# lighttransport/nanort

Measured on NVIDIA H100. Metric: Mrays/sec (primary+1-bounce AO), higher is better.
Workload: dtype f32

## Files before the change

### nanort_b200/csrc/bake.cu

```cuda
#include <algorithm>
#include <mutex>
#include <string>

#include "../../include/nanort_b200_bake.h"
#include "common.cuh"
#include "scan.cuh"
#include "wavefront.cuh"

namespace nrt {

int launch_traverse_texels(const Accel *a, const TexelRays &rays, size_t n, const TexelStore &store, Hit16 *d_by_ray,
                           uint32_t flags, cudaStream_t s);
int launch_traverse_bake(const Accel *a, const BakeAoRays &rays, size_t n, float *d_accum, unsigned long long *d_occluded,
                         uint32_t flags, cudaStream_t s);

namespace {

__global__ void __launch_bounds__(256)
    scatter_texels_kernel(const Hit16 *__restrict__ by_ray, uint32_t n, TexelRays rays, TexelStore store) {
  const uint32_t i = blockIdx.x * blockDim.x + threadIdx.x;
  const bool active = i < n;
  Hit16 h = {0.0f, 0.0f, 1.0e30f, 0xFFFFFFFFu};
  uint32_t texel = 0;
  if (active) {
// ... 3 lines not shown
  store(active, texel, h.t, h.u, h.v, h.prim_id, 1.0e30f);
}

__global__ void __launch_bounds__(256)
    covered_flags_kernel(const Hit16 *__restrict__ rec, uint32_t n, uint32_t n_prims, uint32_t *__restrict__ flags,
                         unsigned long long *info) {
  const uint32_t i = blockIdx.x * blockDim.x + threadIdx.x;
  if (i >= n) return;
  const uint32_t p = rec[i].prim_id;
  flags[i] = p != 0xFFFFFFFFu ? 1u : 0u;
  if (p != 0xFFFFFFFFu && p >= n_prims) info[1] = 1ull;
}

__global__ void __launch_bounds__(256)
    compact_texels_kernel(const Hit16 *__restrict__ rec, uint32_t n, const uint32_t *__restrict__ offs,
                          uint32_t *__restrict__ list, unsigned long long *info) {
  const uint32_t i = blockIdx.x * blockDim.x + threadIdx.x;
  if (i >= n) return;
  const bool covered = rec[i].prim_id != 0xFFFFFFFFu;
  if (covered) list[offs[i]] = i;
  if (i == n - 1) info[0] = (unsigned long long)offs[i] + (covered ? 1ull : 0ull);
}

__global__ void __launch_bounds__(256) bake_rays_kernel(BakeAoRays rays, uint32_t n, Ray36 *__restrict__ out) {
  const uint32_t i = blockIdx.x * blockDim.x + threadIdx.x;
  if (i >= n) return;
  Ray36 r;
  uint32_t texel;
  rays.load(i, r.org[0], r.org[1], r.org[2], r.dir[0], r.dir[1], r.dir[2], r.min_t, r.max_t, &texel);
  r.type = 0;
  out[i] = r;
}

uint32_t scan_launches(uint32_t n) {
  const uint32_t tiles = (n + kScanTile - 1) / kScanTile;
  return n == 0 ? 0u : tiles > 1 ? 2u + scan_launches(tiles) : 1u;
}

}

bool is_triangle_accel(const Accel *a) {
  return a->prim_kind == 0 && !a->d_prim_boxes && a->d_faces && a->d_verts && a->d_pair && a->d_tris_cm;
}

int bake_prepare(Accel *a, const void *d_records, uint32_t n, const char *who, cudaStream_t s, uint32_t **list,
                 uint32_t *n_cov, uint32_t *launches) {
  uint32_t *offs = static_cast<uint32_t *>(a->d_wave);
  *list = offs + n;
  uint32_t *scratch = *list + n;
  unsigned long long *info = reinterpret_cast<unsigned long long *>(a->d_counters) + 2;
  const Hit16 *rec = static_cast<const Hit16 *>(d_records);
  NRT_CUDA(cudaMemsetAsync(info, 0, 2 * sizeof(unsigned long long), s));
  covered_flags_kernel<<<(n + 255) / 256, 256, 0, s>>>(rec, n, a->n_prims, offs, info);
  NRT_CUDA(cudaGetLastError());
  if (const int rc = exclusive_scan_u32_async(offs, offs, n, scratch, s)) return rc;
  compact_texels_kernel<<<(n + 255) / 256, 256, 0, s>>>(rec, n, offs, *list, info);
  NRT_CUDA(cudaGetLastError());
  *launches += 2 + scan_launches(n);
  unsigned long long h[2] = {0, 0};
  NRT_CUDA(cudaMemcpyAsync(h, info, sizeof(h), cudaMemcpyDeviceToHost, s));
  NRT_CUDA(cudaStreamSynchronize(s));
  if (h[1]) {
    set_error(std::string(who) + ": a record's prim_id is not a face of the world accel");
    return NRT_ERR_INVALID;
  }
  *n_cov = (uint32_t)h[0];
  return NRT_OK;
}

}
// ... 240 lines not shown
```

### nanort_b200/csrc/bdpt.cu

```cuda
#include <algorithm>
#include <mutex>
#include <string>

#include "../../include/nanort_b200_scene_bdpt.h"
#include "common.cuh"
#include "radix_sort.cuh"
#include "scan.cuh"
#include "scene.cuh"
#include "wavefront.cuh"

namespace nrt {

int launch_traverse_bdpt_bounce(const Accel *a, const bd::BounceRays &rays, const bd::BounceEpilogue &epi,
                                const unsigned long long *d_count, size_t capacity, uint32_t flags, cudaStream_t s);
int launch_traverse_bdpt_connect(const Accel *a, const bd::ConnRays &rays, const bd::ConnEpilogue &epi,
                                 const unsigned long long *d_count, size_t capacity, uint32_t flags, cudaStream_t s);

namespace {

using namespace bd;

constexpr size_t kWaveBudget = (size_t)512 << 20;

__device__ __forceinline__ void emissive_flag(const Scene &sc, uint32_t id, uint32_t *flag, unsigned long long *info) {
// ... 527 lines not shown
  const uint32_t slot = conns[i].slot, el = conns[i].el, l = el >> 16;
  const size_t ie = (size_t)slot * sp.stride + (el & 0xFFFFu) - 1, il = (size_t)slot * sp.stride + l - 1;
  const float3 pe = f3(sp.eye[ie].position), pl = f3(sp.light[il].position);
  float3 to;
  float dist;
  conn_ray(pe, pl, to, dist);
  const float3 ge = g.geo_normal(sv.eye_inst[ie], sp.eye[ie].prim_id);
  const float3 gl = l == 1 ? g.geo_normal(sv.light_pair[2 * (size_t)slot], sv.light_pair[2 * (size_t)slot + 1])
                           : g.geo_normal(sv.light_inst[il], sp.light[il].prim_id);
  const float3 o = LiftedOrigin{ge}(pe, to);
  Ray36 r;
  r.org[0] = o.x, r.org[1] = o.y, r.org[2] = o.z;
  r.dir[0] = to.x, r.dir[1] = to.y, r.dir[2] = to.z;
  r.min_t = kEps;
  r.max_t = SceneSpawn::plane_max_t(pe.x, pe.y, pe.z, o.x, o.y, o.z, to.x, to.y, to.z, dist, gl.x, gl.y, gl.z);
  r.type = 0;
  rays[i] = r;
}

__global__ void __launch_bounds__(256)
    scene_conn_g_kernel(Conn *__restrict__ conns, uint32_t n, Subpaths sp, const Ray36 *__restrict__ rays,
                        const SceneHit32 *__restrict__ hits, const uint8_t *__restrict__ mask) {
  const uint32_t i = blockIdx.x * blockDim.x + threadIdx.x;
  if (i >= n) return;
  Conn &c = conns[i];
  const uint32_t slot = c.slot, el = c.el;
  const nrt_bdpt_vertex &ev = sp.eye[(size_t)slot * sp.stride + (el & 0xFFFFu) - 1];
  const nrt_bdpt_vertex &lv = sp.light[(size_t)slot * sp.stride + (el >> 16) - 1];
  float3 to;
  float dist;
  conn_ray(f3(ev.position), f3(lv.position), to, dist);
  const bool blocked = mask[i] && hits[i].t < rays[i].max_t;
  conn_finish(c, blocked ? 0.0f : g_term(to, dist, f3(ev.norm), f3(lv.norm)));
}

uint32_t scan_launches(uint32_t n) {
  const uint32_t tiles = (n + kScanTile - 1) / kScanTile;
  return n == 0 ? 0u : tiles > 1 ? 2u + scan_launches(tiles) : 1u;
}

uint32_t max_conns(uint32_t B) { return B * (B + 1) / 2; }

struct Out {
  nrt_bdpt_vertex *eye, *light;
  uint32_t *n_eye, *n_light;
  float *rgb;
  uint32_t *eye_inst, *light_inst, *light_pair;
};

int check_common(const nrt_bdpt_params &p, const char *who) {
  auto bad = [&](const char *why) {
    set_error(std::string(who) + ": " + why);
    return NRT_ERR_INVALID;
  };
  if (p.flags & ~(uint32_t)NRT_TRAVERSE_CONFORMANCE)
    return bad("flags other than NRT_TRAVERSE_CONFORMANCE (calcG needs the nearest distance: no ANY_HIT)");
  if (p.width == 0 || p.height == 0 || p.spp == 0 || p.n_shards == 0 || p.shard >= p.n_shards || p.tile_w == 0 ||
      p.tile_h == 0 || (p.tile_w % 8) != 0 || (p.tile_h % 4) != 0)
    return bad("bad image, sample or tile parameters");
  if ((uint64_t)p.sample0 + p.spp > p.spp_total) return bad("sample0 + spp > spp_total");
  if (p.max_bounces == 0 || p.max_bounces > 64) return bad("max_bounces must lie in [1, 64]");
  return NRT_OK;
}

int check_params(const Accel *a, const nrt_bdpt_params *pp, const char *who) {
  auto bad = [&](const char *why) {
    set_error(std::string(who) + ": " + why);
    return NRT_ERR_INVALID;
  };
  if (!a || !pp) return bad("NULL argument");
  const nrt_bdpt_params &p = *pp;
// ... 521 lines not shown
```

### nanort_b200/csrc/render.cu

```cuda
#include <algorithm>
#include <mutex>
#include <string>

#include "common.cuh"
#include "wavefront.cuh"

namespace nrt {

namespace {

__global__ void __launch_bounds__(256)
    gen_primary_kernel(nrt_ao_params p, unsigned long long slot0, uint32_t count, Wave w,
                       unsigned long long *counters ) {
  uint32_t i = blockIdx.x * blockDim.x + threadIdx.x;
  bool valid = false;
  if (i < count) {
    uint32_t pix, smp;
    if (!slot_to_pixel(p, slot0 + i, pix, smp)) {
      w.pix[i] = 0xFFFFFFFFu;
      w.org_tmin[i] = make_float4(0.f, 0.f, 0.f, 0.f);
      w.dir_tmax[i] = make_float4(0.f, 0.f, -1.f, -1.f);
    } else {
      valid = true;
      smp += p.sample0;
      float dx, dy, dz;
      camera_ray(p.cam, p.width, p.height, p.seed, pix, smp, dx, dy, dz);
      w.pix[i] = pix;
      w.org_tmin[i] = make_float4(p.cam[0], p.cam[1], p.cam[2], p.ray_min_t);
      w.dir_tmax[i] = make_float4(dx, dy, dz, p.ray_max_t);
    }
  }
  const unsigned m = __ballot_sync(0xFFFFFFFFu, valid);
  if ((threadIdx.x & 31) == 0 && m) atomicAdd(counters + 1, (unsigned long long)__popc(m));
}

__global__ void __launch_bounds__(256)
    gen_ao_kernel(nrt_ao_params p, unsigned long long slot0, uint32_t count, Wave w,
// ... 27 lines not shown
    w.ao_dir_tmax[j] = d4;
    w.ao_pix[j] = pix;
  }
}

__global__ void __launch_bounds__(256)
    face_normals_kernel(const float *__restrict__ verts, const uint32_t *__restrict__ faces, uint32_t n,
                        float4 *__restrict__ out) {
  const uint32_t i = blockIdx.x * blockDim.x + threadIdx.x;
  if (i >= n) return;
  float nx, ny, nz, a2;
  geometric_normal(verts, faces, i, nx, ny, nz, a2);
  out[i] = make_float4(nx, ny, nz, 0.0f);
}

__global__ void __launch_bounds__(256)
    accumulate_ao_kernel(Wave w, const unsigned long long *__restrict__ counters, float *__restrict__ accum,
                         unsigned long long *totals ) {
  const unsigned long long n = counters[0];
  const unsigned long long i = (unsigned long long)blockIdx.x * blockDim.x + threadIdx.x;
  bool occluded = false;
  if (i < n) {
    occluded = w.ao_hits[i].prim_id != 0xFFFFFFFFu;
    if (!occluded) atomicAdd(accum + w.ao_pix[i], 1.0f);
  }
  const unsigned m = __ballot_sync(0xFFFFFFFFu, occluded);
  if ((threadIdx.x & 31) == 0 && m) atomicAdd(totals + 1, (unsigned long long)__popc(m));
  if (i == 0) {
    atomicAdd(totals + 0, n);
    atomicAdd(totals + 2, counters[1]);
  }
}

__global__ void fold_wave_counters_kernel(const unsigned long long *counters, unsigned long long *totals) {
  totals[0] += counters[0];
  totals[2] += counters[1];
}

__global__ void __launch_bounds__(256)
    soa_to_aos_kernel(const float4 *__restrict__ org_tmin, const float4 *__restrict__ dir_tmax,
                      const unsigned long long *n_ptr, unsigned long long n, Ray36 *__restrict__ out, uint32_t type) {
  if (n_ptr) n = *n_ptr;
  const unsigned long long i = (unsigned long long)blockIdx.x * blockDim.x + threadIdx.x;
  if (i >= n) return;
  const float4 o = org_tmin[i], d = dir_tmax[i];
  Ray36 r;
  r.org[0] = o.x;
  r.org[1] = o.y;
  r.org[2] = o.z;
  r.dir[0] = d.x;
  r.dir[1] = d.y;
  r.dir[2] = d.z;
  r.min_t = o.w;
  r.max_t = d.w;
  r.type = type;
  out[i] = r;
}

}

int launch_traverse_soa_devcount(const Accel *a, const float4 *d_org_tmin, const float4 *d_dir_tmax,
                                 const unsigned long long *d_count, size_t capacity, Hit16 *d_hits,
                                 const TraceOptions16 &opt, uint32_t flags, cudaStream_t s);
int launch_traverse_camera_fused(Accel *a, const Wave &w, const nrt_ao_params &p, unsigned long long slot0, size_t count,
                                 const float4 *d_face_n, float *d_accum, unsigned long long *d_wave_counters,
                                 const TraceOptions16 &opt, uint32_t flags, cudaStream_t s);
int launch_traverse_ao_fused(const Accel *a, const Wave &w, const unsigned long long *d_count, size_t capacity,
                             float *d_accum, unsigned long long *d_totals, const TraceOptions16 &opt, uint32_t flags,
                             cudaStream_t s);

}

using namespace nrt;

static unsigned long long valid_slots(const nrt_ao_params &p, unsigned long long s0, uint32_t count) {
  const unsigned long long per_tile = (unsigned long long)p.tile_w * p.tile_h * p.spp;
  const uint32_t tiles_x = (p.width + p.tile_w - 1) / p.tile_w;
  unsigned long long total = 0;
  for (unsigned long long k = s0 / per_tile; k < (s0 + count) / per_tile; k++) {
    const unsigned long long tile = k * p.n_shards + p.shard;
    const uint32_t tx = (uint32_t)(tile % tiles_x), ty = (uint32_t)(tile / tiles_x);
    const uint32_t x0 = tx * p.tile_w, y0 = ty * p.tile_h;
    if (x0 >= p.width || y0 >= p.height) continue;
    const uint32_t wv = p.width - x0 < p.tile_w ? p.width - x0 : p.tile_w;
    const uint32_t hv = p.height - y0 < p.tile_h ? p.height - y0 : p.tile_h;
    total += (unsigned long long)wv * hv * p.spp;
  }
  return total;
}

static int run_ao_pass(const nrt_accel *h, const nrt_ao_params *pp, float *d_accum, nrt_ao_result *res, void *stream,
                       Ray36 *dump_primary, Ray36 *dump_ao, uint64_t *n_ao_out) {
  if (!h || !pp || !d_accum) {
    set_error("nrt_render_ao_device: NULL argument");
    return NRT_ERR_INVALID;
  }
  Accel *a = const_cast<Accel *>(reinterpret_cast<const Accel *>(h));
  nrt_ao_params p = *pp;
  if (p.width == 0 || p.height == 0 || p.spp == 0 || p.n_shards == 0 || p.shard >= p.n_shards || p.tile_w == 0 ||
      p.tile_h == 0 || (p.tile_w % 8) != 0 || (p.tile_h % 4) != 0) {
    set_error("nrt_render_ao_device: bad parameters (tiles must be multiples of 8x4 pixels)");
    return NRT_ERR_INVALID;
  }
  if (!a->d_pair || !a->d_tris_cm || !a->d_faces) {
    set_error("nrt_render_ao_device: the AO pass needs a triangle accel");
    return NRT_ERR_INVALID;
  }
  NRT_DEVICE(a->device);
  std::lock_guard<std::mutex> lock(a->host_mu);
  cudaStream_t s = static_cast<cudaStream_t>(stream);
  if (const int rc = wait_previous_pass(a, s)) return rc;
  const RecordOnExit pass_done{a->pass_done, s};
  if (const int rc = ensure_face_normals(a, s)) return rc;
  const uint32_t tiles_x = (p.width + p.tile_w - 1) / p.tile_w, tiles_y = (p.height + p.tile_h - 1) / p.tile_h;
  const uint32_t n_tiles = tiles_x * tiles_y;
  const uint32_t my_tiles = n_tiles > p.shard ? (n_tiles - p.shard + p.n_shards - 1) / p.n_shards : 0;
  const unsigned long long per_tile = (unsigned long long)p.tile_w * p.tile_h * p.spp;
  const unsigned long long total_slots = (unsigned long long)my_tiles * per_tile;

  const unsigned long long kMaxWave = 16ull << 20;
  unsigned long long tiles_per_wave = kMaxWave / per_tile;
  if (tiles_per_wave == 0) tiles_per_wave = 1;
  const unsigned long long cap = std::min<unsigned long long>(total_slots, tiles_per_wave * per_tile);
  const size_t per_ray = 2 * sizeof(float4) + sizeof(Hit16) + 4 + 2 * sizeof(float4) + 4 + sizeof(Hit16);
  const size_t need = (size_t)cap * per_ray + 256;
  if (const int rc = grow_wave(a, need)) return rc;
  Wave w;
  {
    char *b = static_cast<char *>(a->d_wave);
    w.org_tmin = reinterpret_cast<float4 *>(b);
    b += cap * sizeof(float4);
    w.dir_tmax = reinterpret_cast<float4 *>(b);
    b += cap * sizeof(float4);
    w.ao_org_tmin = reinterpret_cast<float4 *>(b);
    b += cap * sizeof(float4);
    w.ao_dir_tmax = reinterpret_cast<float4 *>(b);
    b += cap * sizeof(float4);
    w.hits = reinterpret_cast<Hit16 *>(b);
    b += cap * sizeof(Hit16);
    w.ao_hits = reinterpret_cast<Hit16 *>(b);
    b += cap * sizeof(Hit16);
    w.pix = reinterpret_cast<uint32_t *>(b);
    b += cap * 4;
    w.ao_pix = reinterpret_cast<uint32_t *>(b);
  }
  unsigned long long *wave_ctr = reinterpret_cast<unsigned long long *>(a->d_counters) + 2;
  unsigned long long *totals = reinterpret_cast<unsigned long long *>(a->d_counters) + 4;
  NRT_CUDA(cudaMemsetAsync(totals, 0, 3 * sizeof(unsigned long long), s));

  TraceOptions16 opt = default_trace_options();
  std::vector<cudaEvent_t> ev;
  cudaEvent_t e_begin = nullptr, e_end = nullptr;
  if (res) {
    NRT_CUDA(cudaEventCreate(&e_begin));
    NRT_CUDA(cudaEventCreate(&e_end));
    NRT_CUDA(cudaEventRecord(e_begin, s));
  }
  uint32_t launches = 0, trav_launches = 0;
  unsigned long long dumped_ao = 0, valid_primaries_host = 0;
  const bool fused = !dump_primary && !dump_ao && !(p.flags & NRT_AO_UNFUSED);
  if (!fused && (p.flags & NRT_AO_PACKED_TILES)) {
    set_error("nrt_render_ao_device: NRT_AO_PACKED_TILES needs the fused pass");
    return NRT_ERR_INVALID;
  }
  const uint32_t trav_flags = p.flags & 0xFFFFu;
  int rc = NRT_OK;
  for (unsigned long long s0 = 0; s0 < total_slots && rc == NRT_OK; s0 += cap) {
    const uint32_t count = (uint32_t)std::min<unsigned long long>(cap, total_slots - s0);
    const uint32_t grid = (count + 255) / 256;
    if (cudaMemsetAsync(wave_ctr, 0, 2 * sizeof(unsigned long long), s) != cudaSuccess) {
      rc = NRT_ERR_CUDA;
      break;
    }
    if (!fused) {
      gen_primary_kernel<<<grid, 256, 0, s>>>(p, s0, count, w, wave_ctr);
      launches++;
    }
    cudaEvent_t t0 = nullptr, t1 = nullptr, t2 = nullptr, t3 = nullptr;
    if (res) {
      cudaError_t ee = cudaEventCreate(&t0);
      if (ee == cudaSuccess) ee = cudaEventCreate(&t1);
      if (ee == cudaSuccess) ee = cudaEventCreate(&t2);
      if (ee == cudaSuccess) ee = cudaEventCreate(&t3);
      ev.push_back(t0);
      ev.push_back(t1);
      ev.push_back(t2);
      ev.push_back(t3);
      if (ee != cudaSuccess) {
        rc = cuda_fail(ee, "cudaEventCreate", __FILE__, __LINE__);
        break;
      }
    }
    if (fused) {
      if (res) cudaEventRecord(t0, s);
      rc = launch_traverse_camera_fused(a, w, p, s0, count, a->d_face_n, d_accum, wave_ctr, opt, trav_flags, s);
      if (rc != NRT_OK) break;
      if (res) {
        cudaEventRecord(t1, s);
        cudaEventRecord(t2, s);
      }
      rc = launch_traverse_ao_fused(a, w, wave_ctr, count, d_accum, totals, opt, trav_flags, s);
      if (rc != NRT_OK) break;
      if (res) cudaEventRecord(t3, s);
      fold_wave_counters_kernel<<<1, 1, 0, s>>>(wave_ctr, totals);
      launches += 3;
      trav_launches += 2;
      valid_primaries_host += valid_slots(p, s0, count);
    } else {
      if (dump_primary) {
        soa_to_aos_kernel<<<grid, 256, 0, s>>>(w.org_tmin, w.dir_tmax, nullptr, count, dump_primary + s0, 1u);
        launches++;
      }
      if (res) cudaEventRecord(t0, s);
      rc = launch_traverse_soa(a, w.org_tmin, w.dir_tmax, count, w.hits, opt, trav_flags, s);
      if (rc != NRT_OK) break;
      if (res) cudaEventRecord(t1, s);
      launches++;
      trav_launches++;
      gen_ao_kernel<<<grid, 256, 0, s>>>(p, s0, count, w, a->d_face_n, d_accum, wave_ctr);
      launches++;
      if (dump_ao) {
        unsigned long long n_wave = 0;
        soa_to_aos_kernel<<<grid, 256, 0, s>>>(w.ao_org_tmin, w.ao_dir_tmax, wave_ctr, 0, dump_ao + dumped_ao, 2u);
        launches++;
        cudaMemcpyAsync(&n_wave, wave_ctr, sizeof(n_wave), cudaMemcpyDeviceToHost, s);
        cudaStreamSynchronize(s);
        dumped_ao += n_wave;
      }
      if (res) cudaEventRecord(t2, s);
      rc = launch_traverse_soa_devcount(a, w.ao_org_tmin, w.ao_dir_tmax, wave_ctr, count, w.ao_hits, opt, trav_flags, s);
      if (rc != NRT_OK) break;
      if (res) cudaEventRecord(t3, s);
      launches++;
      trav_launches++;
      accumulate_ao_kernel<<<grid, 256, 0, s>>>(w, wave_ctr, d_accum, totals);
      launches++;
    }
    if (cudaGetLastError() != cudaSuccess) rc = NRT_ERR_CUDA;
// ... 73 lines not shown
```

### nanort_b200/csrc/scan.cuh

```cuda
#pragma once
#include "common.cuh"

namespace nrt {

constexpr int kScanBlock = 256;
constexpr int kScanItems = 8;
constexpr int kScanTile = kScanBlock * kScanItems;

static __global__ void scan_tiles_kernel(const uint32_t *__restrict__ in, uint32_t *__restrict__ out, uint32_t n,
                                         uint32_t *__restrict__ tile_sums) {
  __shared__ uint32_t warp_sums[kScanBlock / 32];
  const uint32_t base = blockIdx.x * kScanTile + threadIdx.x * kScanItems;
  uint32_t v[kScanItems];
  uint32_t sum = 0;
#pragma unroll
  for (int k = 0; k < kScanItems; k++) {
    uint32_t i = base + k;
    v[k] = i < n ? in[i] : 0u;
    sum += v[k];
  }
  uint32_t inc = sum;
  const int lane = threadIdx.x & 31, wid = threadIdx.x >> 5;
#pragma unroll
  for (int o = 1; o < 32; o <<= 1) {
// ... 44 lines not shown
  NRT_CUDA(cudaMalloc(&d_sums, sizeof(uint32_t) * (size_t)(tiles + 1)));
  scan_tiles_kernel<<<tiles, kScanBlock, 0, s>>>(d_in, d_out, n, d_sums);
  NRT_CUDA(cudaGetLastError());
  int rc = NRT_OK;
  if (tiles > 1) {
    uint32_t t2 = 0;
    rc = exclusive_scan_u32(d_sums, d_sums, tiles, total ? &t2 : nullptr, s);
    if (rc == NRT_OK) {
      add_tile_offsets_kernel<<<tiles, kScanBlock, 0, s>>>(d_out, n, d_sums);
      if (cudaGetLastError() != cudaSuccess) rc = NRT_ERR_CUDA;
    }
    if (total) *total = t2;
  } else if (total) {
    if (cudaMemcpyAsync(total, d_sums, sizeof(uint32_t), cudaMemcpyDeviceToHost, s) != cudaSuccess ||
        cudaStreamSynchronize(s) != cudaSuccess)
      rc = NRT_ERR_CUDA;
  }
  if (cudaStreamSynchronize(s) != cudaSuccess) rc = NRT_ERR_CUDA;
  cudaFree(d_sums);
  return rc;
}

static inline size_t scan_scratch_words(uint32_t n) {
  size_t total = 0;
  while (n > 1) {
    uint32_t tiles = (n + kScanTile - 1) / kScanTile;
    total += tiles + 1;
    if (tiles <= 1) break;
    n = tiles;
  }
  return total + 4;
}

static int exclusive_scan_u32_async(const uint32_t *d_in, uint32_t *d_out, uint32_t n, uint32_t *d_scratch,
                                    cudaStream_t s) {
  if (n == 0) return NRT_OK;
  uint32_t tiles = (n + kScanTile - 1) / kScanTile;
  scan_tiles_kernel<<<tiles, kScanBlock, 0, s>>>(d_in, d_out, n, d_scratch);
  NRT_CUDA(cudaGetLastError());
  if (tiles > 1) {
    int rc = exclusive_scan_u32_async(d_scratch, d_scratch, tiles, d_scratch + tiles + 1, s);
    if (rc != NRT_OK) return rc;
    add_tile_offsets_kernel<<<tiles, kScanBlock, 0, s>>>(d_out, n, d_scratch);
    NRT_CUDA(cudaGetLastError());
  }
  return NRT_OK;
}

}
```

### nanort_b200/csrc/traverse.cu

```cuda
#include <float.h>
#include <math_constants.h>

#include "common.cuh"
#include "trav_common.cuh"
#include "wavefront.cuh"
#include "traverse3.cuh"

namespace nrt {

struct AosRays {
  static constexpr int kPayloadWords = 0;
  static constexpr bool kSharedOrigin = false;
  const Ray36 *rays;
  __device__ __forceinline__ void load(size_t i, float &ox, float &oy, float &oz, float &dx, float &dy,
                                       float &dz, float &tmin, float &tmax, uint32_t * = nullptr) const {
    const float *p = reinterpret_cast<const float *>(rays + i);
    ox = __ldcs(p + 0);
    oy = __ldcs(p + 1);
    oz = __ldcs(p + 2);
    dx = __ldcs(p + 3);
    dy = __ldcs(p + 4);
    dz = __ldcs(p + 5);
    tmin = __ldcs(p + 6);
    tmax = __ldcs(p + 7);
// ... 58 lines not shown
    best.v = 0.0f;
    best.prim = 0xFFFFFFFFu;
    reference_walk(nodes, c, min_t, max_t, PackedTriLeaf{tris, c, opt, best}, COUNT ? visits : nullptr);
    if (hits) write_result(hits, mask, i, best, max_t);
  }
  if (COUNT) {
    for (int o = 16; o > 0; o >>= 1) {
      visits[0] += __shfl_down_sync(FULL_MASK, visits[0], o);
      visits[1] += __shfl_down_sync(FULL_MASK, visits[1], o);
    }
    if ((threadIdx.x & 31) == 0) {
      atomicAdd(counts + 0, visits[0]);
      atomicAdd(counts + 1, visits[1]);
    }
  }
}

static int g_sm_count[64] = {0};
int device_sm_count(int device) {
  if (device < 0 || device >= 64) return 132;
  if (g_sm_count[device] == 0) {
    int v = 0;
    if (cudaDeviceGetAttribute(&v, cudaDevAttrMultiProcessorCount, device) != cudaSuccess || v <= 0) v = 132;
    g_sm_count[device] = v;
  }
  return g_sm_count[device];
}

typedef Policy3<10, 24, true, 8, false, 2> DefaultPolicy;
typedef Policy3<9, 32, true, 12, true, 3> CameraPolicy;
typedef PacketPolicy<7, 2> CameraPacketPolicy;
typedef Policy3<10, 20, false, 12, false, 3> IncoherentPolicy;
typedef Policy3<9, 32, false, 12, true, 3> IncoherentCameraPolicy;
typedef Policy3<8, 24, false, 8, true, 2> PathRadiancePolicy;
constexpr size_t kPair128MaxBytes = (size_t)38 << 20;
constexpr size_t kCameraRelMaxBytes = (size_t)24 << 20;

template <class Rays, int DEPTH, bool COUNT, class P, class Epi>
static cudaError_t launch_fast3(const Accel *a, Rays rays, size_t n, Epi epi, const TraceOptions16 &opt,
                                uint32_t flags, unsigned long long *cursor, unsigned long long *d_counts,
                                const unsigned long long *n_ptr, cudaStream_t s) {
  const int sms = device_sm_count(a->device);
  const size_t warps_per_block = kTraverseBlock / 32;
  size_t grid = (size_t)sms * P::kMinBlocks;
  const size_t need_blocks = ((n + 31) / 32 + warps_per_block - 1) / warps_per_block;
  if (grid > need_blocks) grid = need_blocks;
  if (grid == 0) grid = 1;
  const void *nodes = Rays::kSharedOrigin ? static_cast<const void *>(a->d_pair_rel)
                     : P::kPair128        ? static_cast<const void *>(a->d_pair)
                                          : static_cast<const void *>(a->d_wide);
  const TriCM *tris = Rays::kSharedOrigin ? a->d_tris_rel : a->d_tris_cm;
  traverse_fast3_kernel<Rays, DEPTH, COUNT, P, Epi><<<(unsigned)grid, kTraverseBlock, 0, s>>>(
      nodes, tris, rays, n, epi, opt, flags, cursor, d_counts, n_ptr);
  return cudaGetLastError();
}

static bool needs_deep_stack(const Accel *a) { return a->stats.max_tree_depth + 2 > 64u; }

template <class Rays, bool COUNT, class P, class Epi>
static int launch_fast3_cursor(const Accel *a, Rays rays, size_t n, Epi epi, const TraceOptions16 &opt, uint32_t flags,
                               unsigned long long *d_counts, const unsigned long long *n_ptr, cudaStream_t s,
                               unsigned long long *cursor) {
  NRT_CUDA(cudaMemsetAsync(cursor, 0, sizeof(unsigned long long), s));
  cudaError_t e;
  if (needs_deep_stack(a))
    e = launch_fast3<Rays, 512, COUNT, P>(a, rays, n, epi, opt, flags, cursor, d_counts, n_ptr, s);
// ... 105 lines not shown
template <int DEPTH>
static cudaError_t launch_packet(const Accel *a, CameraRays rays, size_t n, const PrimaryToAoEpilogue &epi,
                                 const TraceOptions16 &opt, uint32_t flags, unsigned long long *cursor, cudaStream_t s) {
  typedef CameraUnits<CameraPacketPolicy::kRays> Units;
  const Units units(epi.p);
  const size_t n_units = units.count(n);
  const size_t warps_per_block = kTraverseBlock / 32;
  size_t grid = (size_t)device_sm_count(a->device) * CameraPacketPolicy::kMinBlocks;
  const size_t need_blocks = (n_units + warps_per_block - 1) / warps_per_block;
  if (grid > need_blocks) grid = need_blocks;
  traverse_packet_kernel<CameraRays, Units, DEPTH, CameraPacketPolicy, PrimaryToAoEpilogue>
      <<<(unsigned)grid, kTraverseBlock, 0, s>>>(a->d_pair_rel, a->d_tris_rel, rays, units, n_units, n, epi, opt, flags,
                                                 cursor);
  return cudaGetLastError();
}

static int launch_packet_any(const Accel *a, CameraRays rays, size_t n, const PrimaryToAoEpilogue &epi,
                             const TraceOptions16 &opt, uint32_t flags, cudaStream_t s) {
  if (!a->d_pair_rel || !a->d_tris_rel) {
    set_error("traverse: this accel has no camera-relative traversal layout");
    return NRT_ERR_INVALID;
  }
  return a->ring.run(s, [&](uint32_t k) {
    unsigned long long *cursor = reinterpret_cast<unsigned long long *>(a->d_counters) + 16 + k;
    NRT_CUDA(cudaMemsetAsync(cursor, 0, sizeof(unsigned long long), s));
    const cudaError_t e = needs_deep_stack(a) ? launch_packet<512>(a, rays, n, epi, opt, flags, cursor, s)
                                              : launch_packet<64>(a, rays, n, epi, opt, flags, cursor, s);
    NRT_CUDA(e);
    return NRT_OK;
  });
}

int launch_traverse_camera_fused(Accel *a, const Wave &w, const nrt_ao_params &p, unsigned long long slot0, size_t count,
                                 const float4 *d_face_n, float *d_accum, unsigned long long *d_wave_counters,
                                 const TraceOptions16 &opt, uint32_t flags, cudaStream_t s) {
  PrimaryToAoEpilogue epi{p, w, d_face_n, d_accum, d_wave_counters};
  if (count == 0) return NRT_OK;
  if (a->n_wide * sizeof(PairNode) > kPair128MaxBytes)
    return launch_fast3_any<CameraRaysAbs, false, IncoherentCameraPolicy>(a, CameraRaysAbs(p, slot0), count, epi, opt, flags,
                                                                          nullptr, nullptr, s);
  if (2 * (a->n_wide * sizeof(PairNode) + (size_t)a->n_prims * sizeof(TriCM)) > kCameraRelMaxBytes)
    return launch_fast3_any<CameraRaysAbs, false, CameraPolicy>(a, CameraRaysAbs(p, slot0), count, epi, opt, flags, nullptr,
                                                                nullptr, s);
  const int rc = camera_relative_layout(a, p.cam, s);
  if (rc != NRT_OK) return rc;
  return launch_packet_any(a, CameraRays(p, slot0), count, epi, opt, flags, s);
}

int launch_traverse_ao_fused(const Accel *a, const Wave &w, const unsigned long long *d_count, size_t capacity,
                             float *d_accum, unsigned long long *d_totals, const TraceOptions16 &opt, uint32_t flags,
                             cudaStream_t s) {
  AoAccumulateEpilogue epi{w.ao_pix, d_accum, d_totals};
  if (flags & NRT_TRAVERSE_ANY_HIT)
    return launch_fused<AnyHit<AoAccumulateEpilogue>, IncoherentPolicy>(a, SoaRays{w.ao_org_tmin, w.ao_dir_tmax}, capacity, d_count,
                                                                        AnyHit<AoAccumulateEpilogue>(epi), opt, flags, s);
  return launch_fused<AoAccumulateEpilogue, IncoherentPolicy>(a, SoaRays{w.ao_org_tmin, w.ao_dir_tmax}, capacity, d_count, epi,
                                                              opt, flags, s);
}

int launch_traverse_path_radiance(const Accel *a, const PathShadeEpilogue &epi, const unsigned long long *d_count,
                                  size_t capacity, const TraceOptions16 &opt, uint32_t flags, cudaStream_t s) {
  return launch_fused<PathShadeEpilogue, PathRadiancePolicy>(
      a, SoaRays{epi.q.org_tmin[epi.in], epi.q.dir_tmax[epi.in]}, capacity, d_count, epi, opt, flags, s);
}

int launch_traverse_lightmap_radiance(const Accel *a, const LightmapShadeEpilogue &epi, const unsigned long long *d_count,
                                      size_t capacity, const TraceOptions16 &opt, uint32_t flags, cudaStream_t s) {
  return launch_fused<LightmapShadeEpilogue, PathRadiancePolicy>(
      a, SoaRays{epi.q.org_tmin[epi.in], epi.q.dir_tmax[epi.in]}, capacity, d_count, epi, opt, flags, s);
}

int launch_traverse_path_shadow(const Accel *a, const PathQueues &q, const unsigned long long *d_count,
                                size_t capacity, float *d_accum, const TraceOptions16 &opt, uint32_t flags,
                                cudaStream_t s) {
  ShadowAccumulateEpilogue epi{q.sh_contrib_pix, d_accum};
  if (flags & NRT_TRAVERSE_ANY_HIT)
    return launch_fused<AnyHit<ShadowAccumulateEpilogue>, IncoherentPolicy>(a, SoaRays{q.sh_org_tmin, q.sh_dir_tmax}, capacity,
                                                                            d_count, AnyHit<ShadowAccumulateEpilogue>(epi), opt,
                                                                            flags, s);
  return launch_fused<ShadowAccumulateEpilogue, IncoherentPolicy>(a, SoaRays{q.sh_org_tmin, q.sh_dir_tmax}, capacity, d_count,
                                                                  epi, opt, flags, s);
}

int launch_traverse_texels(const Accel *a, const TexelRays &rays, size_t n, const TexelStore &store, Hit16 *d_by_ray,
                           uint32_t flags, cudaStream_t s) {
  if (n == 0) return NRT_OK;
  const TraceOptions16 opt = default_trace_options();
  if (flags & NRT_TRAVERSE_CONFORMANCE)
    return launch_conf<TexelRays, false>(a, rays, n, d_by_ray, nullptr, opt, flags, nullptr, s);
  return launch_fast3_coherent<TexelRays, false>(a, rays, n, TexelStoreEpilogue{store}, opt, flags, nullptr, nullptr, s);
// ... 78 lines not shown
```

### nanort_b200/csrc/wavefront.cuh

```cuda
#pragma once
#include "../../include/nanort_b200_bdpt.h"
#include "common.cuh"

namespace nrt {

struct Wave {
  float4 *org_tmin;
  float4 *dir_tmax;
  Hit16 *hits;
  uint32_t *pix;
  float4 *ao_org_tmin;
  float4 *ao_dir_tmax;
  uint32_t *ao_pix;
  Hit16 *ao_hits;
};

__device__ __forceinline__ uint32_t hash_u32(uint32_t x) {
  x ^= x >> 16;
  x *= 0x7FEB352Du;
  x ^= x >> 15;
  x *= 0x846CA68Bu;
  x ^= x >> 16;
  return x;
}

__device__ __forceinline__ float rand_ps(uint32_t pix, uint32_t smp, uint32_t dim, uint32_t seed) {
  uint32_t h = hash_u32(pix + seed * 0x9E3779B1u);
  h = hash_u32(h + smp * 0x85EBCA77u + dim * 0xC2B2AE3Du);
  return (float)(h >> 8) * (1.0f / 16777216.0f);
}

struct TileMap {
  uint32_t width, height, spp, sample0, tile_w, tile_h, shard, n_shards;
  uint32_t packed;
};
__host__ __device__ __forceinline__ TileMap tile_map(const nrt_ao_params &p) {
  return TileMap{p.width, p.height, p.spp, p.sample0, p.tile_w, p.tile_h, p.shard, p.n_shards,
                 (p.flags & NRT_AO_PACKED_TILES) ? 1u : 0u};
}
__host__ __device__ __forceinline__ TileMap tile_map(const nrt_path_params &p) {
  return TileMap{p.width, p.height, p.spp, p.sample0, p.tile_w, p.tile_h, p.shard, p.n_shards, 0u};
}

struct FastDiv {
  uint32_t d, mul, shift;
  __host__ __device__ FastDiv() : d(1), mul(0), shift(0xFFFFFFFFu) {}
  __host__ explicit FastDiv(uint32_t dd) : d(dd ? dd : 1), mul(0), shift(0xFFFFFFFFu) {
    if (d > 1) {
// ... 197 lines not shown
  float nx = n.x, ny = n.y, nz = n.z;
  if (nx * d.x + ny * d.y + nz * d.z > 0.0f) {
    nx = -nx;
    ny = -ny;
    nz = -nz;
  }
  float wx, wy, wz;
  ao_direction(nx, ny, nz, pix, smp, p.seed, wx, wy, wz);
  o4 = make_float4(Px, Py, Pz, p.ao_min_t);
  d4 = make_float4(wx, wy, wz, p.ao_max_t);
}

struct StoreHitsEpilogue {
  static constexpr bool kAnyHit = false;
  Hit16 *hits;
  uint8_t *mask;
  __device__ __forceinline__ void operator()(bool retiring, size_t ray_idx, float t, float u, float v, uint32_t prim,
                                             float max_t, const uint32_t *) const {
    if (retiring && hits) {
      const bool hit = t < max_t;
      float4 r = hit ? make_float4(u, v, t, __uint_as_float(prim)) : make_float4(0.0f, 0.0f, max_t, __uint_as_float(0xFFFFFFFFu));
      __stcs(reinterpret_cast<float4 *>(hits) + ray_idx, r);
      if (mask) mask[ray_idx] = hit ? 1 : 0;
    }
  }
};

struct PrimaryToAoEpilogue {
  static constexpr bool kAnyHit = false;
  nrt_ao_params p;
  Wave w;
  const float4 *normals;
  float *accum;
  unsigned long long *counters;
  __device__ __forceinline__ void operator()(bool retiring, size_t ray_idx, float t, float u, float v, uint32_t prim,
                                             float max_t, const uint32_t *payload) const {
    (void)u;
    (void)v;
    bool make = false;
    float4 o4 = make_float4(0.f, 0.f, 0.f, 0.f), d4 = o4;
    uint32_t pix = 0xFFFFFFFFu, acc = 0;
    if (retiring) {
      pix = payload[3];
      if (pix != 0xFFFFFFFFu) {
        const uint32_t smp = payload[4];
        acc = payload[5];
        const float4 ro = make_float4(p.cam[0], p.cam[1], p.cam[2], p.ray_min_t);
        const float4 rd = make_float4(__uint_as_float(payload[0]), __uint_as_float(payload[1]),
                                      __uint_as_float(payload[2]), p.ray_max_t);
        if (t < max_t) {
          make_ao_ray(p, pix, smp, ro, rd, t, prim, normals, o4, d4);
          make = true;
        } else {
          atomicAdd(accum + acc, 1.0f);
        }
      }
    }
    const unsigned m = __ballot_sync(0xFFFFFFFFu, make);
    if (m == 0u) return;
    const int lane = threadIdx.x & 31, leader = __ffs(m) - 1;
    unsigned long long base = 0;
    if (lane == leader) base = atomicAdd(counters, (unsigned long long)__popc(m));
    base = __shfl_sync(0xFFFFFFFFu, base, leader);
    if (make) {
      const unsigned long long j = base + __popc(m & ((1u << lane) - 1u));
      w.ao_org_tmin[j] = o4;
      w.ao_dir_tmax[j] = d4;
      w.ao_pix[j] = acc;
    }
  }
};

struct AoAccumulateEpilogue {
  static constexpr bool kAnyHit = false;
  const uint32_t *ao_pix;
  float *accum;
  unsigned long long *totals;
  __device__ __forceinline__ void operator()(bool retiring, size_t ray_idx, float t, float u, float v, uint32_t prim,
                                             float max_t, const uint32_t *) const {
    (void)u;
    (void)v;
    (void)prim;
    const bool occluded = retiring && (t < max_t);
    if (retiring && !occluded) atomicAdd(accum + ao_pix[ray_idx], 1.0f);
    const unsigned m = __ballot_sync(0xFFFFFFFFu, occluded);
    if (m != 0u && (int)(threadIdx.x & 31) == __ffs(m) - 1) atomicAdd(totals + 1, (unsigned long long)__popc(m));
  }
};

constexpr uint64_t kMaxTexels = 1ull << 31;

struct TexelRays {
  static constexpr int kPayloadWords = 1;
  static constexpr bool kSharedOrigin = false;
  FastDiv width;
  uint32_t height, flip_x, flip_y;
  float r0, r2, usize, vsize, off0, off1, fw, fh;
  __device__ __forceinline__ void load(size_t i, float &ox, float &oy, float &oz, float &dx, float &dy, float &dz,
                                       float &tmin, float &tmax, uint32_t *payload = nullptr) const {
    uint32_t y, x;
    width.divmod((uint32_t)i, y, x);
    ox = r0 + ((float)x * usize + off0) / fw;
    oy = r2 + ((float)y * vsize + off1) / fh;
    oz = 1.0f;
    dx = 0.0f;
    dy = 0.0f;
    dz = -1.0f;
    tmin = 0.0f;
    tmax = 1.0e30f;
    if (payload) payload[0] = dest(x, y);
  }
  __device__ __forceinline__ uint32_t dest(uint32_t x, uint32_t y) const {
    const uint32_t px = flip_x ? width.d - 1u - x : x, py = flip_y ? height - 1u - y : y;
    return py * width.d + px;
  }
};

// ... 870 lines not shown
```

Measured before the change: 7947.

## Bin AO secondary rays by screen tile and direction cell before traversal

The primary-hit epilogue now writes AO rays into per-tile slots using per-tile atomic counters, and tags each ray with an octahedral direction cell. A scan over tile counts and a new shared-memory binning kernel then build an ordering index that groups rays by tile and direction cell. AO traversal reads rays through that index with a new policy. The aim is more coherent AO traversal, at the cost of an extra scan and bin pass, indirect loads, and more wave memory.

```diff
diff --git a/nanort_b200/csrc/bake.cu b/nanort_b200/csrc/bake.cu
--- a/nanort_b200/csrc/bake.cu
+++ b/nanort_b200/csrc/bake.cu
@@ -59,10 +59,6 @@
   out[i] = r;
 }
 
-uint32_t scan_launches(uint32_t n) {
-  const uint32_t tiles = (n + kScanTile - 1) / kScanTile;
-  return n == 0 ? 0u : tiles > 1 ? 2u + scan_launches(tiles) : 1u;
-}
 
 }
 
diff --git a/nanort_b200/csrc/bdpt.cu b/nanort_b200/csrc/bdpt.cu
--- a/nanort_b200/csrc/bdpt.cu
+++ b/nanort_b200/csrc/bdpt.cu
@@ -583,11 +583,6 @@
   conn_ray(f3(ev.position), f3(lv.position), to, dist);
   const bool blocked = mask[i] && hits[i].t < rays[i].max_t;
   conn_finish(c, blocked ? 0.0f : g_term(to, dist, f3(ev.norm), f3(lv.norm)));
-}
-
-uint32_t scan_launches(uint32_t n) {
-  const uint32_t tiles = (n + kScanTile - 1) / kScanTile;
-  return n == 0 ? 0u : tiles > 1 ? 2u + scan_launches(tiles) : 1u;
 }
 
 uint32_t max_conns(uint32_t B) { return B * (B + 1) / 2; }
diff --git a/nanort_b200/csrc/render.cu b/nanort_b200/csrc/render.cu
--- a/nanort_b200/csrc/render.cu
+++ b/nanort_b200/csrc/render.cu
@@ -3,6 +3,7 @@
 #include <string>
 
 #include "common.cuh"
+#include "scan.cuh"
 #include "wavefront.cuh"
 
 namespace nrt {
@@ -96,6 +97,84 @@
   }
 }
 
+constexpr uint32_t kAoBinChunk = 8192;
+constexpr int kAoBinBlock = 512;
+constexpr int bits_for(uint32_t n) { return n > 1u ? 1 + bits_for((n + 1u) / 2u) : 0; }
+constexpr int kAoCellBits = bits_for(kAoCells);
+__global__ void __launch_bounds__(kAoBinBlock, 4)
+    ao_bin_kernel(Wave w, const uint32_t *__restrict__ tile_off, uint32_t tile_slots, uint32_t chunks,
+                  unsigned long long *counters ) {
+  constexpr int kWarps = kAoBinBlock / 32;
+  constexpr uint32_t kPerWarp = kAoBinChunk / kWarps;
+  constexpr uint32_t kCellsPerLane = (kAoCells + 31) / 32;
+  __shared__ uint32_t s_cell4[kAoBinChunk / 4];
+  __shared__ uint32_t s_off[kWarps][kAoCells];
+  __shared__ uint32_t s_out[kAoBinChunk];
+  const uint32_t tile = blockIdx.x / chunks, c0 = (blockIdx.x % chunks) * kAoBinChunk;
+  const uint32_t n_tile = w.ao_tile_n[tile];
+  if (blockIdx.x == gridDim.x - 1 && threadIdx.x == 0) counters[0] = (unsigned long long)tile_off[tile] + n_tile;
+  if (c0 >= n_tile) return;
+  const uint32_t n = min(n_tile - c0, kAoBinChunk);
+  const uint32_t phys0 = tile * tile_slots + c0;
+  const int lane = threadIdx.x & 31, wid = threadIdx.x >> 5;
+  for (uint32_t i = threadIdx.x; i < kWarps * kAoCells; i += kAoBinBlock) (&s_off[0][0])[i] = 0u;
+  __syncthreads();
+  const uint32_t begin = wid * kPerWarp, end = min(n, begin + kPerWarp);
+  const uint32_t *cell4 = reinterpret_cast<const uint32_t *>(w.ao_cell + phys0);
+  constexpr int kLoads = kPerWarp / 128;
+  uint32_t c4[kLoads];
+#pragma unroll
+  for (int k = 0; k < kLoads; k++) {
+    const uint32_t i = begin + 128u * k + 4u * lane;
+    c4[k] = i < end ? __ldcs(cell4 + i / 4) : 0u;
+  }
+#pragma unroll
+  for (int k = 0; k < kLoads; k++) {
+    const uint32_t i = begin + 128u * k + 4u * lane;
+    if (i < end) s_cell4[i / 4] = c4[k];
+    for (uint32_t b = 0; b < 4 && i + b < end; b++) atomicAdd(&s_off[wid][(c4[k] >> (8 * b)) & 0xFFu], 1u);
+  }
+  __syncthreads();
+  if (wid == 0) {
+    uint32_t sum = 0;
+    for (uint32_t c = lane * kCellsPerLane; c < min((lane + 1) * kCellsPerLane, kAoCells); c++)
+      for (int k = 0; k < kWarps; k++) sum += s_off[k][c];
+    uint32_t inc = sum;
+#pragma unroll
+    for (int o = 1; o < 32; o <<= 1) {
+      const uint32_t x = __shfl_up_sync(0xFFFFFFFFu, inc, o);
+      if (lane >= o) inc += x;
+    }
+    uint32_t base = inc - sum;
+    for (uint32_t c = lane * kCellsPerLane; c < min((lane + 1) * kCellsPerLane, kAoCells); c++)
+      for (int k = 0; k < kWarps; k++) {
+        const uint32_t m = s_off[k][c];
+        s_off[k][c] = base;
+        base += m;
+      }
+  }
+  __syncthreads();
+  const uint8_t *s_cell = reinterpret_cast<const uint8_t *>(s_cell4);
+  for (uint32_t i0 = begin; i0 < end; i0 += 32) {
+    const uint32_t i = i0 + (uint32_t)lane;
+    const bool valid = i < end;
+    const uint32_t cell = valid ? s_cell[i] : 0u;
+    unsigned peers = __ballot_sync(0xFFFFFFFFu, valid);
+#pragma unroll
+    for (int b = 0; b < kAoCellBits; b++) {
+      const unsigned ones = __ballot_sync(0xFFFFFFFFu, (cell >> b) & 1u);
+      peers &= ((cell >> b) & 1u) ? ones : ~ones;
+    }
+    if (valid) s_out[s_off[wid][cell] + __popc(peers & ((1u << lane) - 1u))] = phys0 + i;
+    __syncwarp();
+    if (valid && lane == __ffs(peers) - 1) s_off[wid][cell] += __popc(peers);
+    __syncwarp();
+  }
+  __syncthreads();
+  uint32_t *out = w.ao_order + tile_off[tile] + c0;
+  for (uint32_t i = threadIdx.x; i < n; i += kAoBinBlock) out[i] = s_out[i];
+}
+
 __global__ void fold_wave_counters_kernel(const unsigned long long *counters, unsigned long long *totals) {
   totals[0] += counters[0];
   totals[2] += counters[1];
@@ -127,8 +206,8 @@
                                  const unsigned long long *d_count, size_t capacity, Hit16 *d_hits,
                                  const TraceOptions16 &opt, uint32_t flags, cudaStream_t s);
 int launch_traverse_camera_fused(Accel *a, const Wave &w, const nrt_ao_params &p, unsigned long long slot0, size_t count,
-                                 const float4 *d_face_n, float *d_accum, unsigned long long *d_wave_counters,
-                                 const TraceOptions16 &opt, uint32_t flags, cudaStream_t s);
+                                 const float4 *d_face_n, float *d_accum, const TraceOptions16 &opt, uint32_t flags,
+                                 cudaStream_t s);
 int launch_traverse_ao_fused(const Accel *a, const Wave &w, const unsigned long long *d_count, size_t capacity,
                              float *d_accum, unsigned long long *d_totals, const TraceOptions16 &opt, uint32_t flags,
                              cudaStream_t s);
@@ -186,10 +265,12 @@
   unsigned long long tiles_per_wave = kMaxWave / per_tile;
   if (tiles_per_wave == 0) tiles_per_wave = 1;
   const unsigned long long cap = std::min<unsigned long long>(total_slots, tiles_per_wave * per_tile);
-  const size_t per_ray = 2 * sizeof(float4) + sizeof(Hit16) + 4 + 2 * sizeof(float4) + 4 + sizeof(Hit16);
-  const size_t need = (size_t)cap * per_ray + 256;
+  const uint32_t wave_tiles = (uint32_t)(cap / per_tile);
+  const size_t per_ray = 2 * sizeof(float4) + sizeof(Hit16) + 4 + 2 * sizeof(float4) + 4 + sizeof(Hit16) + 4 + 1;
+  const size_t need = (size_t)cap * per_ray + (2 * (size_t)wave_tiles + scan_scratch_words(wave_tiles)) * 4 + 256;
   if (const int rc = grow_wave(a, need)) return rc;
   Wave w;
+  uint32_t *tile_off, *scan_scratch;
   {
     char *b = static_cast<char *>(a->d_wave);
     w.org_tmin = reinterpret_cast<float4 *>(b);
@@ -207,6 +288,16 @@
     w.pix = reinterpret_cast<uint32_t *>(b);
     b += cap * 4;
     w.ao_pix = reinterpret_cast<uint32_t *>(b);
+    b += cap * 4;
+    w.ao_order = reinterpret_cast<uint32_t *>(b);
+    b += cap * 4;
+    w.ao_tile_n = reinterpret_cast<uint32_t *>(b);
+    b += (size_t)wave_tiles * 4;
+    tile_off = reinterpret_cast<uint32_t *>(b);
+    b += (size_t)wave_tiles * 4;
+    scan_scratch = reinterpret_cast<uint32_t *>(b);
+    b += scan_scratch_words(wave_tiles) * 4;
+    w.ao_cell = reinterpret_cast<uint8_t *>(b);
   }
   unsigned long long *wave_ctr = reinterpret_cast<unsigned long long *>(a->d_counters) + 2;
   unsigned long long *totals = reinterpret_cast<unsigned long long *>(a->d_counters) + 4;
@@ -232,7 +323,8 @@
   for (unsigned long long s0 = 0; s0 < total_slots && rc == NRT_OK; s0 += cap) {
     const uint32_t count = (uint32_t)std::min<unsigned long long>(cap, total_slots - s0);
     const uint32_t grid = (count + 255) / 256;
-    if (cudaMemsetAsync(wave_ctr, 0, 2 * sizeof(unsigned long long), s) != cudaSuccess) {
+    if (cudaMemsetAsync(wave_ctr, 0, 2 * sizeof(unsigned long long), s) != cudaSuccess ||
+        (fused && cudaMemsetAsync(w.ao_tile_n, 0, (size_t)wave_tiles * 4, s) != cudaSuccess)) {
       rc = NRT_ERR_CUDA;
       break;
     }
@@ -257,17 +349,20 @@
     }
     if (fused) {
       if (res) cudaEventRecord(t0, s);
-      rc = launch_traverse_camera_fused(a, w, p, s0, count, a->d_face_n, d_accum, wave_ctr, opt, trav_flags, s);
+      rc = launch_traverse_camera_fused(a, w, p, s0, count, a->d_face_n, d_accum, opt, trav_flags, s);
       if (rc != NRT_OK) break;
-      if (res) {
-        cudaEventRecord(t1, s);
-        cudaEventRecord(t2, s);
-      }
+      if (res) cudaEventRecord(t1, s);
+      const uint32_t tiles = (uint32_t)((count + per_tile - 1) / per_tile);
+      const uint32_t chunks = (uint32_t)((per_tile + kAoBinChunk - 1) / kAoBinChunk);
+      rc = exclusive_scan_u32_async(w.ao_tile_n, tile_off, tiles, scan_scratch, s);
+      if (rc != NRT_OK) break;
+      ao_bin_kernel<<<tiles * chunks, kAoBinBlock, 0, s>>>(w, tile_off, (uint32_t)per_tile, chunks, wave_ctr);
+      if (res) cudaEventRecord(t2, s);
       rc = launch_traverse_ao_fused(a, w, wave_ctr, count, d_accum, totals, opt, trav_flags, s);
       if (rc != NRT_OK) break;
       if (res) cudaEventRecord(t3, s);
       fold_wave_counters_kernel<<<1, 1, 0, s>>>(wave_ctr, totals);
-      launches += 3;
+      launches += 4 + scan_launches(tiles);
       trav_launches += 2;
       valid_primaries_host += valid_slots(p, s0, count);
     } else {
diff --git a/nanort_b200/csrc/scan.cuh b/nanort_b200/csrc/scan.cuh
--- a/nanort_b200/csrc/scan.cuh
+++ b/nanort_b200/csrc/scan.cuh
@@ -100,6 +100,11 @@
   return total + 4;
 }
 
+static inline uint32_t scan_launches(uint32_t n) {
+  const uint32_t tiles = (n + kScanTile - 1) / kScanTile;
+  return n == 0 ? 0u : tiles > 1 ? 2u + scan_launches(tiles) : 1u;
+}
+
 static int exclusive_scan_u32_async(const uint32_t *d_in, uint32_t *d_out, uint32_t n, uint32_t *d_scratch,
                                     cudaStream_t s) {
   if (n == 0) return NRT_OK;
diff --git a/nanort_b200/csrc/traverse.cu b/nanort_b200/csrc/traverse.cu
--- a/nanort_b200/csrc/traverse.cu
+++ b/nanort_b200/csrc/traverse.cu
@@ -114,6 +114,7 @@
 typedef PacketPolicy<7, 2> CameraPacketPolicy;
 typedef Policy3<10, 20, false, 12, false, 3> IncoherentPolicy;
 typedef Policy3<9, 32, false, 12, true, 3> IncoherentCameraPolicy;
+typedef Policy3<10, 24, false, 12, true, 3> BinnedAoPolicy;
 typedef Policy3<8, 24, false, 8, true, 2> PathRadiancePolicy;
 constexpr size_t kPair128MaxBytes = (size_t)38 << 20;
 constexpr size_t kCameraRelMaxBytes = (size_t)24 << 20;
@@ -285,9 +286,9 @@
 }
 
 int launch_traverse_camera_fused(Accel *a, const Wave &w, const nrt_ao_params &p, unsigned long long slot0, size_t count,
-                                 const float4 *d_face_n, float *d_accum, unsigned long long *d_wave_counters,
-                                 const TraceOptions16 &opt, uint32_t flags, cudaStream_t s) {
-  PrimaryToAoEpilogue epi{p, w, d_face_n, d_accum, d_wave_counters};
+                                 const float4 *d_face_n, float *d_accum, const TraceOptions16 &opt, uint32_t flags,
+                                 cudaStream_t s) {
+  PrimaryToAoEpilogue epi{p, w, d_face_n, d_accum, FastDiv(p.tile_w * p.tile_h * p.spp)};
   if (count == 0) return NRT_OK;
   if (a->n_wide * sizeof(PairNode) > kPair128MaxBytes)
     return launch_fast3_any<CameraRaysAbs, false, IncoherentCameraPolicy>(a, CameraRaysAbs(p, slot0), count, epi, opt, flags,
@@ -304,11 +305,11 @@
                              float *d_accum, unsigned long long *d_totals, const TraceOptions16 &opt, uint32_t flags,
                              cudaStream_t s) {
   AoAccumulateEpilogue epi{w.ao_pix, d_accum, d_totals};
+  const OrderedSoaRays rays{w.ao_order, w.ao_org_tmin, w.ao_dir_tmax};
   if (flags & NRT_TRAVERSE_ANY_HIT)
-    return launch_fused<AnyHit<AoAccumulateEpilogue>, IncoherentPolicy>(a, SoaRays{w.ao_org_tmin, w.ao_dir_tmax}, capacity, d_count,
+    return launch_fused<AnyHit<AoAccumulateEpilogue>, IncoherentPolicy>(a, rays, capacity, d_count,
                                                                         AnyHit<AoAccumulateEpilogue>(epi), opt, flags, s);
-  return launch_fused<AoAccumulateEpilogue, IncoherentPolicy>(a, SoaRays{w.ao_org_tmin, w.ao_dir_tmax}, capacity, d_count, epi,
-                                                              opt, flags, s);
+  return launch_fused<AoAccumulateEpilogue, BinnedAoPolicy>(a, rays, capacity, d_count, epi, opt, flags, s);
 }
 
 int launch_traverse_path_radiance(const Accel *a, const PathShadeEpilogue &epi, const unsigned long long *d_count,
diff --git a/nanort_b200/csrc/wavefront.cuh b/nanort_b200/csrc/wavefront.cuh
--- a/nanort_b200/csrc/wavefront.cuh
+++ b/nanort_b200/csrc/wavefront.cuh
@@ -13,7 +13,37 @@
   float4 *ao_dir_tmax;
   uint32_t *ao_pix;
   Hit16 *ao_hits;
-};
+  uint32_t *ao_tile_n;
+  uint8_t *ao_cell;
+  uint32_t *ao_order;
+};
+
+constexpr uint32_t kAoCellGrid = 8;
+constexpr uint32_t kAoCells = kAoCellGrid * kAoCellGrid;
+__device__ __forceinline__ uint32_t ao_dir_cell(float x, float y, float z) {
+  const float s = __fdividef(1.0f, fabsf(x) + fabsf(y) + fabsf(z));
+  float u = x * s, v = y * s;
+  if (z < 0.0f) {
+    const float fu = (1.0f - fabsf(v)) * (u >= 0.0f ? 1.0f : -1.0f);
+    v = (1.0f - fabsf(u)) * (v >= 0.0f ? 1.0f : -1.0f);
+    u = fu;
+  }
+  const float g = 0.5f * (float)kAoCellGrid;
+  const uint32_t cu = min(__float2uint_rz((u + 1.0f) * g), kAoCellGrid - 1u);
+  const uint32_t cv = min(__float2uint_rz((v + 1.0f) * g), kAoCellGrid - 1u);
+  return cv * kAoCellGrid + cu;
+}
+
+__device__ __forceinline__ unsigned same_key_lanes(unsigned among, uint32_t key) {
+  unsigned peers = 0u;
+  while (among) {
+    const uint32_t k = __shfl_sync(0xFFFFFFFFu, key, __ffs(among) - 1);
+    const unsigned same = __ballot_sync(0xFFFFFFFFu, key == k) & among;
+    if (key == k) peers = same;
+    among &= ~same;
+  }
+  return peers;
+}
 
 __device__ __forceinline__ uint32_t hash_u32(uint32_t x) {
   x ^= x >> 16;
@@ -277,14 +307,14 @@
   Wave w;
   const float4 *normals;
   float *accum;
-  unsigned long long *counters;
+  FastDiv tile_slots;
   __device__ __forceinline__ void operator()(bool retiring, size_t ray_idx, float t, float u, float v, uint32_t prim,
                                              float max_t, const uint32_t *payload) const {
     (void)u;
     (void)v;
     bool make = false;
     float4 o4 = make_float4(0.f, 0.f, 0.f, 0.f), d4 = o4;
-    uint32_t pix = 0xFFFFFFFFu, acc = 0;
+    uint32_t pix = 0xFFFFFFFFu, acc = 0, tile = 0xFFFFFFFFu;
     if (retiring) {
       pix = payload[3];
       if (pix != 0xFFFFFFFFu) {
@@ -296,6 +326,7 @@
         if (t < max_t) {
           make_ao_ray(p, pix, smp, ro, rd, t, prim, normals, o4, d4);
           make = true;
+          tile = tile_slots.div((uint32_t)ray_idx);
         } else {
           atomicAdd(accum + acc, 1.0f);
         }
@@ -303,16 +334,40 @@
     }
     const unsigned m = __ballot_sync(0xFFFFFFFFu, make);
     if (m == 0u) return;
-    const int lane = threadIdx.x & 31, leader = __ffs(m) - 1;
-    unsigned long long base = 0;
-    if (lane == leader) base = atomicAdd(counters, (unsigned long long)__popc(m));
-    base = __shfl_sync(0xFFFFFFFFu, base, leader);
+    const unsigned peers = same_key_lanes(m, tile);
+    const int lane = threadIdx.x & 31, leader = __ffs(peers) - 1;
+    uint32_t base = 0;
+    if (make && lane == leader) base = atomicAdd(w.ao_tile_n + tile, (uint32_t)__popc(peers));
+    base = __shfl_sync(0xFFFFFFFFu, base, leader < 0 ? lane : leader);
     if (make) {
-      const unsigned long long j = base + __popc(m & ((1u << lane) - 1u));
+      const size_t j = (size_t)tile * tile_slots.d + base + __popc(peers & ((1u << lane) - 1u));
       w.ao_org_tmin[j] = o4;
       w.ao_dir_tmax[j] = d4;
       w.ao_pix[j] = acc;
-    }
+      w.ao_cell[j] = (uint8_t)ao_dir_cell(d4.x, d4.y, d4.z);
+    }
+  }
+};
+
+struct OrderedSoaRays {
+  static constexpr int kPayloadWords = 1;
+  static constexpr bool kSharedOrigin = false;
+  const uint32_t *order;
+  const float4 *org_tmin;
+  const float4 *dir_tmax;
+  __device__ __forceinline__ void load(size_t i, float &ox, float &oy, float &oz, float &dx, float &dy, float &dz,
+                                       float &tmin, float &tmax, uint32_t *payload) const {
+    const uint32_t j = __ldcs(order + i);
+    const float4 o = __ldcs(org_tmin + j), d = __ldcs(dir_tmax + j);
+    ox = o.x;
+    oy = o.y;
+    oz = o.z;
+    tmin = o.w;
+    dx = d.x;
+    dy = d.y;
+    dz = d.z;
+    tmax = d.w;
+    payload[0] = j;
   }
 };
 
@@ -321,13 +376,13 @@
   const uint32_t *ao_pix;
   float *accum;
   unsigned long long *totals;
-  __device__ __forceinline__ void operator()(bool retiring, size_t ray_idx, float t, float u, float v, uint32_t prim,
-                                             float max_t, const uint32_t *) const {
+  __device__ __forceinline__ void operator()(bool retiring, size_t, float t, float u, float v, uint32_t prim,
+                                             float max_t, const uint32_t *payload) const {
     (void)u;
     (void)v;
     (void)prim;
     const bool occluded = retiring && (t < max_t);
-    if (retiring && !occluded) atomicAdd(accum + ao_pix[ray_idx], 1.0f);
+    if (retiring && !occluded) atomicAdd(accum + ao_pix[payload[0]], 1.0f);
     const unsigned m = __ballot_sync(0xFFFFFFFFu, occluded);
     if (m != 0u && (int)(threadIdx.x & 31) == __ffs(m) - 1) atomicAdd(totals + 1, (unsigned long long)__popc(m));
   }
```

New measurement: 8172 (median of 6 runs). +2.8%, better.
